# alex-petrenko/megaverse

Measured on NVIDIA H100. Metric: agent obs/sec (whole box), higher is better.
Workload: dtype f32

## Files before the change

### megaverse_b200/capi.py

```python
import ctypes as C
import os

import numpy as np

_PKG = os.path.dirname(os.path.abspath(__file__))
LIB_PATH = os.environ.get("MV_B200_LIB") or os.path.join(_PKG, "libmegaverse_b200.so")
_lib = None

MV_OK, MV_ERR_ARG, MV_ERR_CUDA, MV_ERR_CAPACITY, MV_ERR_STATE = 0, -1, -2, -3, -4
MV_END_NONE, MV_END_TIME, MV_END_SOLVED, MV_END_REQUESTED = 0, 1, 2, 3
MV_SEG_NONE, MV_SEG_STATIC, MV_SEG_TERRAIN, MV_SEG_OBJECT, MV_SEG_AGENT, MV_SEG_REWARD = 0, 1, 2, 3, 4, 5
MAX_OBJECTS, MAX_AGENTS, MAX_CAND = 128, 8, 96
MV_FAULT_ENVELOPE, MV_FAULT_CAND_OVERFLOW = 16, 32
CUDA_STREAM_LEGACY = 0x1


class MegaverseError(RuntimeError):
    def __init__(self, code, msg):
        super().__init__("megaverse_b200 error %d: %s" % (code, msg))
        self.code = code


def lib():
    global _lib
# ... 402 lines not shown
    def stream(self):
        p = C.c_void_p()
        self._ck(lib().mv_stream(self._h, C.byref(p)))
        return p.value

    def get_reward_shaping(self, env, agent):
        keys = (C.c_char_p * 32)()
        vals = (C.c_float * 32)()
        n = C.c_int()
        self._ck(lib().mv_get_reward_shaping(self._h, env, agent, keys, vals, 32, C.byref(n)))
        return {keys[i].decode(): float(vals[i]) for i in range(n.value)}

    def set_reward_shaping(self, env, agent, rs):
        keys = (C.c_char_p * max(1, len(rs)))(*[k.encode() for k in rs])
        vals = (C.c_float * max(1, len(rs)))(*[float(v) for v in rs.values()])
        self._ck(lib().mv_set_reward_shaping(self._h, env, agent, keys, vals, len(rs)))

    def faults(self):
        f = C.c_int32()
        self._ck(lib().mv_faults(self._h, C.byref(f)))
        return f.value

    def fault_word(self):
        f = C.c_int32()
        lib().mv_fault_word.argtypes = [C.c_void_p, C.POINTER(C.c_int32)]
        self._ck(lib().mv_fault_word(self._h, C.byref(f)))
        return f.value

    def kernel_launches(self):
        n = C.c_int64()
        self._ck(lib().mv_kernel_launches(self._h, C.byref(n)))
        return n.value

    def step_profile(self, enable=True, read=True):
        out = np.zeros((self.E, 16), dtype=np.uint32)
        lib().mv_debug_step_profile.argtypes = [C.c_void_p, C.c_void_p, C.c_int]
        self._ck(lib().mv_debug_step_profile(self._h, out.ctypes.data if read else None, 1 if enable else 0))
        return out

    def static_cap(self):
        lib().mv_debug_static_cap.argtypes = [C.c_void_p]
        return int(lib().mv_debug_static_cap(self._h))

    def raster_config(self):
        out = (C.c_int32 * 4)()
        lib().mv_debug_raster_config.argtypes = [C.c_void_p, C.c_void_p]
        self._ck(lib().mv_debug_raster_config(self._h, out))
        return {"grid": out[0], "ctas_per_sm": out[1], "smem": out[2], "bands": out[3]}

    def raster_stats(self, enable=True, read=True):
        out = (C.c_ulonglong * 16)()
        lib().mv_debug_raster_stats.argtypes = [C.c_void_p, C.c_void_p, C.c_int]
        self._ck(lib().mv_debug_raster_stats(self._h, out if read else None, 1 if enable else 0))
        names = ["work_items", "instances", "visible_instances", "items", "clipped_items", "triangles", "batches", "sub_passes", "cyc_head", "cyc_tma_wait", "cyc_instance", "cyc_item", "cyc_tile", "cyc_total"]
        return {n: int(out[i]) for i, n in enumerate(names)}

    def states_create(self, rows):
        sid = C.c_int()
        self._ck(lib().mv_states_create(self._h, int(rows), C.byref(sid)))
        return sid.value

    def states_save(self, store, envs, rows):
        e, r = np.ascontiguousarray(envs, dtype=np.int32), np.ascontiguousarray(rows, dtype=np.int32)
        assert e.size == r.size
        self._ck(lib().mv_states_save(self._h, int(store), e.ctypes.data, r.ctypes.data, e.size))

    def states_load(self, store, rows, envs):
        r, e = np.ascontiguousarray(rows, dtype=np.int32), np.ascontiguousarray(envs, dtype=np.int32)
        assert e.size == r.size
        self._ck(lib().mv_states_load(self._h, int(store), r.ctypes.data, e.ctypes.data, e.size))

    def states_destroy(self, store):
        self._ck(lib().mv_states_destroy(self._h, int(store)))

    def state_row_bytes(self):
        n = C.c_int64()
        self._ck(lib().mv_state_row_bytes(self._h, C.byref(n)))
        return n.value

    def last_kernel_ms(self):
        out = (C.c_float * 2)()
        self._ck(lib().mv_last_kernel_ms(self._h, out))
        return float(out[0]), float(out[1])

    def last_final_ms(self):
        out = C.c_float()
        self._ck(lib().mv_last_final_ms(self._h, C.byref(out)))
        return float(out.value)

    def _dump(self, fn, env, dtype, cap=1 << 16):
        out = np.zeros(cap, dtype=dtype)
        n = getattr(lib(), fn)(self._h, env, out.ctypes.data, cap)
        if n < -8:
            return self._dump(fn, env, dtype, -n)
        if n < 0:
            self._ck(n)
        return out[:n].copy()

    def level(self, env):
        return self._dump("mv_debug_get_level", env, np.int32)

    def state(self, env):
        return self._dump("mv_debug_get_state", env, np.float32)

    def voxels(self, env):
        return self._dump("mv_debug_get_voxels", env, np.int32).reshape(-1, 4)

# ... 107 lines not shown
```

### megaverse_b200/csrc/raster_view.cuh

```cuda
#pragma once
#include "dev_math.cuh"
#include "mesh_tables.inc"
#include "mv_types.h"

namespace mvr {
using namespace dm;

struct __align__(16) TriCover {
    long long C[3];
    int32_t A[3], B[3];
    float z[3];
    float invArea;
    uint32_t key;
    int32_t flags;
    uint32_t bx, by;
};
struct __align__(16) TriShade {
    float rw[3];
    float p[9];
    float n[9];
    float diffuse[3];
};
static_assert(sizeof(TriCover) == 80 && sizeof(TriShade) == 96, "triangle record layout");

#ifndef MV_VIEW_THREADS
#define MV_VIEW_THREADS 256
#endif
#ifndef MV_VIEW_MIN_CTAS
#define MV_VIEW_MIN_CTAS 2
#endif
constexpr int kThreads = MV_VIEW_THREADS;
constexpr int kWarps = kThreads / 32;
#ifndef MV_VIEW_INST_CHUNK
#define MV_VIEW_INST_CHUNK 128
#endif
constexpr int kInstChunk = MV_VIEW_INST_CHUNK;
static_assert(kInstChunk <= kThreads && kInstChunk <= 128, "one thread per instance of a chunk; slow-list entries keep 7 bits of it");
constexpr int kXfWords = 23;
constexpr int kClipVerts = 6;
constexpr int kSmallList = 128;
#ifndef MV_SMALL_AREA
#define MV_SMALL_AREA 4
#endif
constexpr int kSmallArea = MV_SMALL_AREA;
constexpr int kIdxBits = 10;
constexpr uint32_t kStaleIdx = (1u << kIdxBits) - 1u;
constexpr int kMaxTriCap = int(kStaleIdx);
constexpr int kKeyBits = 32 - kIdxBits;
constexpr int kMaxInstancesPerEnv = (1 << (kKeyBits - 7)) - 1;
static_assert(MV_CAPSULE_TRIS <= 128 && MV_SPHERE_TRIS <= 128 && MV_CONE_TRIS <= 128 && MV_CYLINDER_TRIS <= 128, "triangle-in-mesh index needs 7 bits");

constexpr int kVBox = 0, kVCapsule = kVBox + MV_BOX_VERTS, kVSphere = kVCapsule + MV_CAPSULE_VERTS, kVCone = kVSphere + MV_SPHERE_VERTS,
              kVCylinder = kVCone + MV_CONE_VERTS, kMeshVerts = kVCylinder + MV_CYLINDER_VERTS;
constexpr int kICapsule = 0, kISphere = kICapsule + MV_CAPSULE_TRIS * 3, kICone = kISphere + MV_SPHERE_TRIS * 3, kICylinder = kICone + MV_CONE_TRIS * 3,
              kMeshIdx = kICylinder + MV_CYLINDER_TRIS * 3;

struct ViewParams {
    const MvInstance *instances;
    const int32_t *instCounts;
    const float *views;
    int instStride;
    uint8_t *obs;
    float *depth;
    uint16_t *seg;
    uint32_t *workCounter;
    uint32_t counterBase;
    const uint32_t *ready;
    uint32_t readyStamp;
    unsigned long long *stats;
    uint32_t *viewCost;
    uint32_t *order;
    uint32_t *exitCounter;
    unsigned long long *spill;
    int spillStride;
    int viewBase, N;
    int A, W, H;
    int bands, bandRows;
    int triCap;
    float p00, p11, p22, p32;
    const uint8_t *envMask;
    const int32_t *camEnv;
    uint32_t *rangeCount;
    int numEnvs;
};

struct SmemLayout { uint32_t stage, cover, shade, xf, off, frag, small, meshV, meshI, clip, slow, sched, misc, total; };
struct ViewMisc {
    float view[16];
    int32_t counts[8];
    int32_t nTris;
    int32_t nValid;
    int32_t tileCtr;
    uint32_t claim;
    int32_t prefetched;
    int32_t lastCta;
    int32_t wsum[kWarps];
    int32_t nSlow[2];
    uint32_t stat[8];
    alignas(8) unsigned long long bar[2];
    unsigned long long itemStart;
};
__host__ __device__ inline SmemLayout smemLayout(int triCap) {
    SmemLayout L;
    uint32_t o = 0;
    L.stage = o; o += 2u * kInstChunk * uint32_t(sizeof(MvInstance));
    L.cover = o; o += uint32_t(triCap) * uint32_t(sizeof(TriCover));
    L.shade = o; o += uint32_t(triCap) * uint32_t(sizeof(TriShade));
    L.xf = o; o += uint32_t(kXfWords) * kInstChunk * 4u;
    L.off = o; o += (kInstChunk + 4u) * 4u;
    L.frag = o; o += uint32_t(kWarps) * 128u * 8u;
    L.meshV = o; o += uint32_t(kMeshVerts) * 6u * 4u;
    L.meshI = o; o += (uint32_t(kMeshIdx) + 15u) & ~15u;
    L.clip = L.frag;
    L.small = o; o += uint32_t(kWarps) * kSmallList * 2u;
    L.slow = o; o += 2u * kThreads * 2u;
    L.sched = o; o += 256u * 4u;
    L.misc = o; o += (uint32_t(sizeof(ViewMisc)) + 15u) & ~15u;
    L.total = o;
    return L;
}

__device__ __forceinline__ uint32_t smemAddrOf(const void *p) { return uint32_t(__cvta_generic_to_shared(p)); }
__device__ __forceinline__ void mbarInit(unsigned long long *bar, int count) {
    asm volatile("mbarrier.init.shared::cta.b64 [%0], %1;" ::"r"(smemAddrOf(bar)), "r"(count));
    asm volatile("fence.mbarrier_init.release.cluster;" ::: "memory");
}
__device__ __forceinline__ void mbarExpectTx(unsigned long long *bar, uint32_t bytes) {
    asm volatile("mbarrier.arrive.expect_tx.shared::cta.b64 _, [%0], %1;" ::"r"(smemAddrOf(bar)), "r"(bytes) : "memory");
}
__device__ __forceinline__ void bulkG2S(void *dst, const void *src, uint32_t bytes, unsigned long long *bar) {
    asm volatile("cp.async.bulk.shared::cluster.global.mbarrier::complete_tx::bytes [%0], [%1], %2, [%3];" ::"r"(smemAddrOf(dst)), "l"(src), "r"(bytes),
                 "r"(smemAddrOf(bar))
                 : "memory");
}
__device__ __forceinline__ void mbarWait(unsigned long long *bar, uint32_t parity) {
    uint32_t done;
    do {
        asm volatile(
            "{\n"
            ".reg .pred p;\n"
            "mbarrier.try_wait.parity.shared::cta.b64 p, [%1], %2;\n"
            "selp.u32 %0, 1, 0, p;\n"
            "}\n"
            : "=r"(done)
            : "r"(smemAddrOf(bar)), "r"(parity)
            : "memory");
    } while (!done);
}

__constant__ float c_palette[22][3];

struct ClipVert { float cx, cy, cz, cw, px, py, pz, nx, ny, nz; };
static_assert(sizeof(ClipVert) == 40, "ClipVert is ten floats");

__device__ __forceinline__ ClipVert lerpVert(const ClipVert &a, const ClipVert &b, float t) {
    ClipVert o;
    o.cx = a.cx + t * (b.cx - a.cx); o.cy = a.cy + t * (b.cy - a.cy); o.cz = a.cz + t * (b.cz - a.cz); o.cw = a.cw + t * (b.cw - a.cw);
    o.px = a.px + t * (b.px - a.px); o.py = a.py + t * (b.py - a.py); o.pz = a.pz + t * (b.pz - a.pz);
    o.nx = a.nx + t * (b.nx - a.nx); o.ny = a.ny + t * (b.ny - a.ny); o.nz = a.nz + t * (b.nz - a.nz);
    return o;
}
__device__ __forceinline__ int32_t snapSub(float v) { return int32_t(floorf(v * 256.0f + 0.5f)); }

struct SetupCtx {
    TriCover *cover;
    TriShade *shade;
    int32_t *nTris;
    int32_t *nValid;
    int triCap;
    int W, H;
    int rowLo, rowHi;
};
__device__ __forceinline__ int nthFace(unsigned mask, int n) {
    int face = 0, seen = 0;
#pragma unroll
    for (int f = 0; f < 6; ++f) {
        const int bit = int(mask >> f) & 1;
        if (bit && seen == n) face = f;
        seen += bit;
    }
    return face;
}
__device__ __forceinline__ int reserveTris(const SetupCtx &cx, int n) {
    int base;
    asm volatile("atom.shared.add.s32 %0, [%1], %2;" : "=r"(base) : "r"(smemAddrOf(cx.nTris)), "r"(n) : "memory");
    if (base + n <= cx.triCap) return base;
    asm volatile("red.shared.min.s32 [%0], %1;" ::"r"(smemAddrOf(cx.nValid)), "r"(base) : "memory");
    return -1;
}

struct ScreenVert { int32_t sx, sy; float sz, rw; };
__device__ __forceinline__ ScreenVert projectVert(const ClipVert &v, float hw, float hh) {
    ScreenVert o;
    const float r = 1.0f / v.cw;
    o.rw = r;
    o.sx = snapSub((v.cx * r) * hw + hw);
    o.sy = snapSub((v.cy * r) * hh + hh);
    o.sz = v.cz * r;
    return o;
}
__device__ __forceinline__ bool snapOutOfRange(const ScreenVert &a, const ScreenVert &b, const ScreenVert &c) {
    constexpr long long kSnapMax = 1518500249ll;
    const long long x0 = a.sx, x1 = b.sx, x2 = c.sx, y0 = a.sy, y1 = b.sy, y2 = c.sy;
    const long long ax = max(llabs(x0), max(llabs(x1), llabs(x2))), ay = max(llabs(y0), max(llabs(y1), llabs(y2)));
    const long long dx = max(x0, max(x1, x2)) - min(x0, min(x1, x2)), dy = max(y0, max(y1, y2)) - min(y0, min(y1, y2));
    return ax > kSnapMax || ay > kSnapMax || dx >= (1ll << 31) || dy >= (1ll << 31);
}

struct TriBox { long long area2; uint32_t bx, by; };
__device__ __forceinline__ bool triBox(const SetupCtx &cx, const ScreenVert &a, const ScreenVert &b, const ScreenVert &c, TriBox &o) {
    o.area2 = (long long)(b.sx - a.sx) * (long long)(c.sy - a.sy) - (long long)(b.sy - a.sy) * (long long)(c.sx - a.sx);
    if (o.area2 >= 0) return false;
    const int32_t minx = min(a.sx, min(b.sx, c.sx)), maxx = max(a.sx, max(b.sx, c.sx));
    const int32_t miny = min(a.sy, min(b.sy, c.sy)), maxy = max(a.sy, max(b.sy, c.sy));
    const int px0 = max(0, (minx - 128 + 255) >> 8), px1 = min(cx.W - 1, (maxx - 128) >> 8);
    const int py0 = max(0, (miny - 128 + 255) >> 8), py1 = min(cx.H - 1, (maxy - 128) >> 8);
    if (px0 > px1 || py0 > py1) return false;
    if (py0 > cx.rowHi || py1 < cx.rowLo) return false;
    o.bx = uint32_t(px0) | (uint32_t(px1) << 16);
    o.by = uint32_t(py0) | (uint32_t(py1) << 16);
    return true;
}
template <bool FAST>
__device__ __forceinline__ void writeTri(const SetupCtx &cx, int slot, const ClipVert &va, const ClipVert &vb, const ClipVert &vc, const ScreenVert &a,
                                         const ScreenVert &b, const ScreenVert &c, const TriBox &tb, int colorTag, uint32_t key) {
    const int color = colorTag & 0xffff;
    TriCover cv;
    TriShade s;
    const int32_t sxs[3] = {a.sx, b.sx, c.sx}, sys[3] = {a.sy, b.sy, c.sy};
    int tl = 0;
    long long worst = 0;
    const long long wsub = (long long)cx.W * 256, hsub = (long long)cx.H * 256;
#pragma unroll
    for (int e = 0; e < 3; ++e) {
        const int ia = (e + 1) % 3, ib = (e + 2) % 3;
        const long long dx = (long long)sxs[ib] - sxs[ia], dy = (long long)sys[ib] - sys[ia];
        const bool topleft = (dy == 0 && dx < 0) || dy > 0;
        cv.A[e] = int32_t(dy);
        cv.B[e] = int32_t(-dx);
        cv.C[e] = dx * sys[ia] - dy * sxs[ia] - (topleft ? 0 : 1);
        tl |= topleft ? (1 << e) : 0;
        const long long bound = llabs(dy) * wsub + llabs(dx) * hsub + llabs(cv.C[e]);
        worst = bound > worst ? bound : worst;
    }
    cv.z[0] = a.sz; cv.z[1] = b.sz; cv.z[2] = c.sz;
    s.rw[0] = a.rw; s.rw[1] = b.rw; s.rw[2] = c.rw;
    s.p[0] = va.px; s.p[1] = va.py; s.p[2] = va.pz; s.p[3] = vb.px; s.p[4] = vb.py; s.p[5] = vb.pz; s.p[6] = vc.px; s.p[7] = vc.py; s.p[8] = vc.pz;
    s.n[0] = va.nx; s.n[1] = va.ny; s.n[2] = va.nz; s.n[3] = vb.nx; s.n[4] = vb.ny; s.n[5] = vb.nz; s.n[6] = vc.nx; s.n[7] = vc.ny; s.n[8] = vc.nz;
    const bool flat = va.nx == vb.nx && va.ny == vb.ny && va.nz == vb.nz && va.nx == vc.nx && va.ny == vc.ny && va.nz == vc.nz;
    if (FAST && flat) {
        const float inv = rsqrtf(va.nx * va.nx + va.ny * va.ny + va.nz * va.nz);
        s.n[0] = va.nx * inv; s.n[1] = va.ny * inv; s.n[2] = va.nz * inv;
    }
    cv.invArea = 1.0f / float(-tb.area2);
    cv.key = key;
    cv.flags = tl | (worst < (1ll << 30) ? 8 : 0) | (flat ? 16 : 0) | (colorTag & int(0xffff0000u));
    cv.bx = tb.bx;
    cv.by = tb.by;
    s.diffuse[0] = c_palette[color][0]; s.diffuse[1] = c_palette[color][1]; s.diffuse[2] = c_palette[color][2];
    cx.cover[slot] = cv;
    cx.shade[slot] = s;
}

__device__ __forceinline__ void vertPosition(ClipVert &cv, const float mv[12], const float *vp, float p00, float p11, float p22, float p32) {
    { float acc = 0.0f; acc += mv[0] * vp[0]; acc += mv[3] * vp[1]; acc += mv[6] * vp[2]; acc += mv[9] * 1.0f; cv.px = acc; }
    { float acc = 0.0f; acc += mv[1] * vp[0]; acc += mv[4] * vp[1]; acc += mv[7] * vp[2]; acc += mv[10] * 1.0f; cv.py = acc; }
    { float acc = 0.0f; acc += mv[2] * vp[0]; acc += mv[5] * vp[1]; acc += mv[8] * vp[2]; acc += mv[11] * 1.0f; cv.pz = acc; }
    cv.cx = cv.px * p00;
    cv.cy = cv.py * p11;
    cv.cz = cv.pz * p22 + p32;
    cv.cw = -cv.pz;
}
__device__ __forceinline__ void vertNormal(ClipVert &cv, const float nm[9], const float *vp) {
    cv.nx = nm[0] * vp[3] + nm[3] * vp[4] + nm[6] * vp[5];
    cv.ny = nm[1] * vp[3] + nm[4] * vp[4] + nm[7] * vp[5];
    cv.nz = nm[2] * vp[3] + nm[5] * vp[4] + nm[8] * vp[5];
}
__device__ __forceinline__ ClipVert makeVert(const float mv[12], const float nm[9], const float *vp, float p00, float p11, float p22, float p32) {
    ClipVert cv;
    vertPosition(cv, mv, vp, p00, p11, p22, p32);
    vertNormal(cv, nm, vp);
    return cv;
}

__device__ __forceinline__ bool insideNearFar(const ClipVert &v) { return v.cz >= 0.0f && (v.cw - v.cz) >= 0.0f; }
__device__ __forceinline__ unsigned sideOutcode(const ClipVert &v) {
    return (v.cx > v.cw ? 1u : 0u) | (v.cx < -v.cw ? 2u : 0u) | (v.cy > v.cw ? 4u : 0u) | (v.cy < -v.cw ? 8u : 0u);
}

enum SetupResult { kSetupDone = 0, kSetupFull = 1, kSetupClip = 2 };

template <bool FAST, bool RANGE = false>
__device__ __forceinline__ SetupResult setupItem(const SetupCtx &cx, ClipVert &v0, ClipVert &v1, ClipVert &v2, ClipVert &v3, int nTri, const float nm[9], const float *vp0,
                                                 const float *vp1, const float *vp2, const float *vp3, int color, uint32_t keyBase,
                                                 uint32_t *rangeCount = nullptr) {
    if (sideOutcode(v0) & sideOutcode(v1) & sideOutcode(v2) & sideOutcode(v3)) return kSetupDone;
    if (!(insideNearFar(v0) && insideNearFar(v1) && insideNearFar(v2) && insideNearFar(v3))) {
        if (v0.cz < 0.0f && v1.cz < 0.0f && v2.cz < 0.0f && v3.cz < 0.0f) return kSetupDone;
        if ((v0.cw - v0.cz) < 0.0f && (v1.cw - v1.cz) < 0.0f && (v2.cw - v2.cz) < 0.0f && (v3.cw - v3.cz) < 0.0f) return kSetupDone;
        return kSetupClip;
    }
    const float hw = float(cx.W) * 0.5f, hh = float(cx.H) * 0.5f;
    const ScreenVert s0 = projectVert(v0, hw, hh), s1 = projectVert(v1, hw, hh), s2 = projectVert(v2, hw, hh);
    ScreenVert s3 = s2;
    if (nTri == 2) s3 = projectVert(v3, hw, hh);
    TriBox b0, b1;
    const bool vis0 = triBox(cx, s0, s1, s2, b0), vis1 = nTri == 2 && triBox(cx, s0, s2, s3, b1);
    const int n = (vis0 ? 1 : 0) + (vis1 ? 1 : 0);
    auto countWide = [&] {
        const uint32_t wide = (snapOutOfRange(s0, s1, s2) ? 1u : 0u) + (nTri == 2 && snapOutOfRange(s0, s2, s3) ? 1u : 0u);
        if (wide && rangeCount) atomicAdd(rangeCount, wide);
    };
    if (!n) {
        if (RANGE) countWide();
        return kSetupDone;
    }
    int slot = reserveTris(cx, n);
    if (slot < 0) return kSetupFull;
    if (RANGE) countWide();
    vertNormal(v0, nm, vp0); vertNormal(v1, nm, vp1); vertNormal(v2, nm, vp2); vertNormal(v3, nm, vp3);
#pragma unroll 1
    for (int t = 0; t < 2; ++t) {
        if (!(t ? vis1 : vis0)) continue;
        const ClipVert vb = t ? v2 : v1, vc = t ? v3 : v2;
        const ScreenVert sb = t ? s2 : s1, sc = t ? s3 : s2;
        const TriBox tb = t ? b1 : b0;
        writeTri<FAST>(cx, slot++, v0, vb, vc, s0, sb, sc, tb, color, keyBase + uint32_t(t));
    }
    return kSetupDone;
}

__device__ __forceinline__ int clipNearFar(float *bufA, float *bufB, int c, unsigned groupMask) {
    float *src = bufA, *dst = bufB;
    int n = 3;
    for (int plane = 0; plane < 2; ++plane) {
        int m = 0;
        for (int i = 0; i < n; ++i) {
            const int i1 = i + 1 == n ? 0 : i + 1;
            const float az = src[i * 10 + 2], aw = src[i * 10 + 3], bz = src[i1 * 10 + 2], bw = src[i1 * 10 + 3];
            const float da = plane == 0 ? az : aw - az;
            const float db = plane == 0 ? bz : bw - bz;
            const bool ina = da >= 0.0f, inb = db >= 0.0f;
            float a = 0.0f, b = 0.0f;
            if (c < 10) { a = src[i * 10 + c]; b = src[i1 * 10 + c]; }
            if (ina) { if (c < 10) dst[m * 10 + c] = a; ++m; }
            if (ina != inb) {
                float val;
                if (ina) { const float t = da / (da - db); val = a + t * (b - a); }
                else { const float t = db / (db - da); val = b + t * (a - b); }
                if (c < 10) dst[m * 10 + c] = val;
                ++m;
            }
        }
        __syncwarp(groupMask);
        n = m;
        float *sw = src; src = dst; dst = sw;
        if (n < 3) return 0;
    }
    return n;
}

__device__ __forceinline__ bool instanceMayBeVisible(const M4 &mv, float by, float p00, float p11) {
    const float l0 = sqrtf(mv.c[0] * mv.c[0] + mv.c[1] * mv.c[1] + mv.c[2] * mv.c[2]);
    const float l1 = sqrtf(mv.c[4] * mv.c[4] + mv.c[5] * mv.c[5] + mv.c[6] * mv.c[6]);
    const float l2 = sqrtf(mv.c[8] * mv.c[8] + mv.c[9] * mv.c[9] + mv.c[10] * mv.c[10]);
    const float r = (l0 + by * l1 + l2) * 1.001f + 1e-3f;
    const float x = mv.c[12], y = mv.c[13], z = mv.c[14];
    if (-z - 0.01f < -r) return false;
    const float ix = rsqrtf(p00 * p00 + 1.0f), iy = rsqrtf(p11 * p11 + 1.0f);
    const float ax = fabsf(p00), ay = fabsf(p11);
    if ((-ax * x - z) * ix < -r || (ax * x - z) * ix < -r) return false;
    if ((-ay * y - z) * iy < -r || (ay * y - z) * iy < -r) return false;
    return true;
// ... 422 lines not shown

    if (tid == 0) { M.claim = claimWork<ITEMS>(P, total); M.prefetched = 0; }
    for (;;) {
        const long long tc0 = P.stats ? clock64() : 0;
        long long tcWait = 0, tcInst = 0, tcItem = 0;
        __syncthreads();
        const uint32_t claim = M.claim;
        const bool prefetched = M.prefetched != 0;
        if (claim >= total) break;
        const int vrel = int(claim / uint32_t(bands)), band = int(claim - uint32_t(vrel) * uint32_t(bands));
        const int view = P.viewBase + vrel;
        const int env = CAM ? P.camEnv[vrel] : view / P.A;
        const bool live = !CAM || (env >= 0 && env < P.numEnvs);
        const int rowLo = band * P.bandRows, rowHi = min(P.H, rowLo + P.bandRows) - 1;
        const int bandTiles = tilesX * ((rowHi - rowLo + 1) >> 2);
        const MvInstance *inst = P.instances + size_t(env) * size_t(P.instStride);

        if (tid == 0) {
            if (P.ready && !prefetched) {
                const uint32_t *flag = P.ready + env;
                uint32_t v;
                while (true) {
                    asm volatile("ld.acquire.gpu.global.u32 %0, [%1];" : "=r"(v) : "l"(flag) : "memory");
                    if (v == P.readyStamp) break;
                    __nanosleep(200);
                }
                asm volatile("fence.proxy.async;" ::: "memory");
            }
            M.itemStart = (unsigned long long)clock64();
            M.nTris = 0;
            M.nValid = 0x7fffffff;
            M.tileCtr = 0;
            M.nSlow[0] = 0; M.nSlow[1] = 0;
            for (int q = 0; q < 8; ++q) M.stat[q] = 0;
        }
        __syncthreads();
        if (!prefetched) {
            if (tid < 16) M.view[tid] = __ldcg(P.views + size_t(view) * 16 + tid);
            else if (tid < 24) M.counts[tid - 16] = live ? __ldcg(P.instCounts + env * 8 + (tid - 16)) : 0;
            __syncthreads();
        }
        const int nInst = M.counts[1];
        const int nChunks = (nInst + kInstChunk - 1) / kInstChunk;
        if (tid == 0 && nChunks > 0 && !prefetched) {
            const uint32_t bytes = uint32_t(min(nInst, kInstChunk)) * uint32_t(sizeof(MvInstance));
            mbarExpectTx(&M.bar[0], bytes);
            bulkG2S(stage, inst, bytes, &M.bar[0]);
        }
        M4 viewM;
#pragma unroll
        for (int i = 0; i < 16; ++i) viewM.c[i] = M.view[i];

        SetupCtx cx;
        cx.cover = cover; cx.shade = shade; cx.nTris = &M.nTris; cx.nValid = &M.nValid; cx.triCap = P.triCap; cx.W = P.W; cx.H = P.H; cx.rowLo = rowLo; cx.rowHi = rowHi;
        int batch = 0, parity = 0;
        const long long tc1 = P.stats ? clock64() : 0;

        for (int c = 0; c < nChunks; ++c) {
            const int buf = c & 1;
            const int cBase = c * kInstChunk, cCnt = min(kInstChunk, nInst - cBase);
            const long long tw0 = P.stats ? clock64() : 0;
            mbarWait(&M.bar[buf], phase[buf]);
            phase[buf] ^= 1u;
            const long long tw1 = P.stats ? clock64() : 0;
            tcWait += tw1 - tw0;
            if (tid == 0 && c + 1 < nChunks) {
                const int nCnt = min(kInstChunk, nInst - (cBase + kInstChunk));
                const uint32_t bytes = uint32_t(nCnt) * uint32_t(sizeof(MvInstance));
                mbarExpectTx(&M.bar[buf ^ 1], bytes);
                bulkG2S(stage + (buf ^ 1) * kInstChunk, inst + cBase + kInstChunk, bytes, &M.bar[buf ^ 1]);
            }
            int items = 0;
            if (tid < cCnt) {
                const float4 *src = reinterpret_cast<const float4 *>(stage + buf * kInstChunk + tid);
                const float4 c0 = src[0], c1 = src[1], c2 = src[2], c3 = src[3], c4 = src[4];
                M4 model;
                model.c[0] = c0.x; model.c[1] = c0.y; model.c[2] = c0.z; model.c[3] = c0.w;
                model.c[4] = c1.x; model.c[5] = c1.y; model.c[6] = c1.z; model.c[7] = c1.w;
                model.c[8] = c2.x; model.c[9] = c2.y; model.c[10] = c2.z; model.c[11] = c2.w;
                model.c[12] = c3.x; model.c[13] = c3.y; model.c[14] = c3.z; model.c[15] = c3.w;
                const int mesh = __float_as_int(c4.x), color = __float_as_int(c4.y);
                const M4 mv = mul4(viewM, model);
                int meta = mesh;
                if (instanceMayBeVisible(mv, mesh == 1 ? 2.0f : 1.0f, P.p00, P.p11)) {
                    float nm[9];
                    const float det = normalMatrix(mv, nm);
                    const bool mirrored = !(det > 0.0f);
                    if (mirrored) meta |= 1 << 16;
                    if (mesh == 0) {
                        int mask = mirrored ? 63 : 0;
#pragma unroll
                        for (int face = 0; face < 6; ++face) {
                            const float *fn = meshV + (face * 4) * 6 + 3;
                            const float cxv = mv.c[12] + (fn[0] * mv.c[0] + fn[1] * mv.c[4] + fn[2] * mv.c[8]);
                            const float cyv = mv.c[13] + (fn[0] * mv.c[1] + fn[1] * mv.c[5] + fn[2] * mv.c[9]);
                            const float czv = mv.c[14] + (fn[0] * mv.c[2] + fn[1] * mv.c[6] + fn[2] * mv.c[10]);
                            const float nxv = nm[0] * fn[0] + nm[3] * fn[1] + nm[6] * fn[2];
                            const float nyv = nm[1] * fn[0] + nm[4] * fn[1] + nm[7] * fn[2];
                            const float nzv = nm[2] * fn[0] + nm[5] * fn[1] + nm[8] * fn[2];
                            const float d = nxv * cxv + nyv * cyv + nzv * czv;
                            if (!(d > 1e-3f * sqrtf((nxv * nxv + nyv * nyv + nzv * nzv) * (cxv * cxv + cyv * cyv + czv * czv)))) mask |= 1 << face;
                        }
                        items = __popc(mask);
                        meta |= mask << 8;
                    } else {
                        items = mesh == 1 ? MV_CAPSULE_TRIS : (mesh == 2 ? MV_SPHERE_TRIS : (mesh == 3 ? MV_CONE_TRIS : MV_CYLINDER_TRIS));
                    }
                    if (items) {
#pragma unroll
                        for (int col = 0; col < 4; ++col)
#pragma unroll
                            for (int row = 0; row < 3; ++row) xf[(col * 3 + row) * kInstChunk + tid] = mv.c[col * 4 + row];
#pragma unroll
                        for (int q = 0; q < 9; ++q) xf[(12 + q) * kInstChunk + tid] = nm[q];
                        xf[21 * kInstChunk + tid] = __int_as_float(color | (__float_as_int(c4.z) << 16));
                    }
                }
                xf[22 * kInstChunk + tid] = __int_as_float(meta);
                if (P.stats && items) atomicAdd(&M.stat[2], 1u);
            }
            {
                int incl = items;
#pragma unroll
                for (int d = 1; d < 32; d <<= 1) {
                    const int up = __shfl_up_sync(0xffffffffu, incl, d);
                    if (lane >= d) incl += up;
                }
                if (lane == 31) M.wsum[warp] = incl;
                __syncthreads();
                int prefix = 0, totalItems = 0;
#pragma unroll
                for (int w = 0; w < kWarps; ++w) { const int s = M.wsum[w]; if (w < warp) prefix += s; totalItems += s; }
                if (tid < kInstChunk) off[tid] = prefix + incl - items;
                if (tid == 0) off[kInstChunk] = totalItems;
                __syncthreads();
            }
            const int totalItems = off[kInstChunk];
            const long long tw2 = P.stats ? clock64() : 0;
            tcInst += tw2 - tw1;
            if (P.stats && tid == 0) { M.stat[1] += uint32_t(cCnt); M.stat[3] += uint32_t(totalItems); }
            for (int ibase = 0; ibase < totalItems; ibase += kThreads, parity ^= 1) {
                const int j = ibase + tid;
                uint16_t *slowList = slowAll + parity * kThreads;
                if (tid == 0) { M.nSlow[parity ^ 1] = 0; if (P.stats) M.stat[7] += 1; }
                bool pending = j < totalItems, pushed = false, again = false;
                for (;;) {
                    if (pending) {
                        int lo = 0, hi = cCnt - 1;
                        while (lo < hi) {
                            const int mid = (lo + hi + 1) >> 1;
                            if (off[mid] <= j) lo = mid; else hi = mid - 1;
                        }
                        const int i = lo, sub = j - off[i];
                        float mv[12], nm[9];
#pragma unroll
                        for (int q = 0; q < 12; ++q) mv[q] = xf[q * kInstChunk + i];
#pragma unroll
                        for (int q = 0; q < 9; ++q) nm[q] = xf[(12 + q) * kInstChunk + i];
                        const int color = __float_as_int(xf[21 * kInstChunk + i]);
                        const int meta = __float_as_int(xf[22 * kInstChunk + i]);
                        const int mesh = meta & 255;
                        const uint32_t ii = uint32_t(cBase + i);
                        ClipVert cvt[4];
                        const float *vpn[4];
                        int nTri;
                        uint32_t keyBase;
                        bool facesAway = false;
                        if (mesh == 0) {
                            const int face = nthFace(unsigned(meta >> 8) & 63u, sub);
#pragma unroll
                            for (int k = 0; k < 4; ++k) vpn[k] = meshV + (face * 4 + k) * 6;
                            nTri = 2; keyBase = ii * 128u + uint32_t(face) * 2u + 1u;
                        } else {
                            const int vBase = mesh == 1 ? kVCapsule : (mesh == 2 ? kVSphere : (mesh == 3 ? kVCone : kVCylinder));
                            const int iBase = mesh == 1 ? kICapsule : (mesh == 2 ? kISphere : (mesh == 3 ? kICone : kICylinder));
#pragma unroll
                            for (int k = 0; k < 3; ++k) vpn[k] = meshV + (vBase + int(meshI[iBase + sub * 3 + k])) * 6;
                            vpn[3] = vpn[2];
                            nTri = 1; keyBase = ii * 128u + uint32_t(sub) + 1u;
#ifndef MV_NO_MESH_PRECULL
                            if (!(meta & (1 << 16))) {
                                const float t0 = mv[9], t1 = mv[10], t2 = mv[11];
                                const float ex = -(nm[0] * t0 + nm[1] * t1 + nm[2] * t2), ey = -(nm[3] * t0 + nm[4] * t1 + nm[5] * t2), ez = -(nm[6] * t0 + nm[7] * t1 + nm[8] * t2);
                                const float *pa = vpn[0], *pb = vpn[1], *pc = vpn[2];
                                const float ux = pb[0] - pa[0], uy = pb[1] - pa[1], uz = pb[2] - pa[2], vx = pc[0] - pa[0], vy = pc[1] - pa[1], vz = pc[2] - pa[2];
                                const float nx = uy * vz - uz * vy, ny = uz * vx - ux * vz, nz = ux * vy - uy * vx;
                                const float dx = ex - pa[0], dy = ey - pa[1], dz = ez - pa[2];
                                const float sd = nx * dx + ny * dy + nz * dz;
                                facesAway = sd < 0.0f && sd * sd > 4e-4f * ((nx * nx + ny * ny + nz * nz) * (dx * dx + dy * dy + dz * dz));
                            }
#endif
                        }
                        SetupResult res = kSetupDone;
                        if (!facesAway) {
#pragma unroll
                            for (int k = 0; k < 4; ++k) vertPosition(cvt[k], mv, vpn[k], P.p00, P.p11, P.p22, P.p32);
                            res = setupItem<FAST, CAM>(cx, cvt[0], cvt[1], cvt[2], cvt[3], nTri, nm, vpn[0], vpn[1], vpn[2], vpn[3], color, keyBase,
                                                       CAM && band == 0 ? P.rangeCount : nullptr);
                        }
                        pending = res == kSetupFull;
                        if (res == kSetupClip) {
                            int at;
                            asm volatile("atom.shared.add.s32 %0, [%1], 1;" : "=r"(at) : "r"(smemAddrOf(&M.nSlow[parity])) : "memory");
                            slowList[at] = uint16_t(i | (sub << 7));
                            pushed = true;
                        }
                    }
                    const bool any = __syncthreads_or((pending || pushed) ? 1 : 0) || again;
                    pushed = false;
                    if (!any) break;
                    bool slowFull = false;
                    const int nSlow = M.nSlow[parity];
                    if (P.stats && tid == 0 && !again) M.stat[4] += uint32_t(nSlow);
                    for (int sidx = warp; sidx < nSlow; sidx += kWarps) {
                        const int e = slowList[sidx];
                        if (e & 0x8000) continue;
                        const int i = e & 127, sub = (e >> 7) & 127;
                        float mv[12], nm[9];
#pragma unroll
                        for (int q = 0; q < 12; ++q) mv[q] = xf[q * kInstChunk + i];
#pragma unroll
                        for (int q = 0; q < 9; ++q) nm[q] = xf[(12 + q) * kInstChunk + i];
                        const int color = __float_as_int(xf[21 * kInstChunk + i]);
                        const int meta = __float_as_int(xf[22 * kInstChunk + i]);
                        const int mesh = meta & 255;
                        const uint32_t ii = uint32_t(cBase + i);
                        ClipVert *poly0 = clipScratch, *poly1 = clipScratch + kClipVerts, *tmp0 = clipScratch + 2 * kClipVerts, *tmp1 = clipScratch + 3 * kClipVerts;
                        int nSrc;
                        uint32_t keyBase;
                        if (mesh == 0) {
                            const int face = nthFace(unsigned(meta >> 8) & 63u, sub);
                            nSrc = 2; keyBase = ii * 128u + uint32_t(face) * 2u + 1u;
                            if (lane < 4) {
                                const ClipVert v = makeVert(mv, nm, meshV + (face * 4 + lane) * 6, P.p00, P.p11, P.p22, P.p32);
                                if (lane == 0) { poly0[0] = v; poly1[0] = v; }
                                else if (lane == 1) poly0[1] = v;
                                else if (lane == 2) { poly0[2] = v; poly1[1] = v; }
                                else poly1[2] = v;
                            }
                        } else {
                            const int vBase = mesh == 1 ? kVCapsule : (mesh == 2 ? kVSphere : (mesh == 3 ? kVCone : kVCylinder));
                            const int iBase = mesh == 1 ? kICapsule : (mesh == 2 ? kISphere : (mesh == 3 ? kICone : kICylinder));
                            nSrc = 1; keyBase = ii * 128u + uint32_t(sub) + 1u;
                            if (lane < 3) poly0[lane] = makeVert(mv, nm, meshV + (vBase + int(meshI[iBase + sub * 3 + lane])) * 6, P.p00, P.p11, P.p22, P.p32);
                        }
                        __syncwarp();
                        int nv = 0;
                        if ((lane >> 4) < nSrc)
                            nv = clipNearFar(reinterpret_cast<float *>(lane >> 4 ? poly1 : poly0), reinterpret_cast<float *>(lane >> 4 ? tmp1 : tmp0), lane & 15,
                                             0xffffu << (lane & 16));
                        __syncwarp();
                        const int n0 = __shfl_sync(0xffffffffu, nv, 0), n1 = __shfl_sync(0xffffffffu, nv, 16);
                        const int t = lane / 3, k = lane - t * 3 + 1;
                        const ClipVert *pp = t ? poly1 : poly0;
                        bool vis = false, wide = false;
                        TriBox tb;
                        ScreenVert sa, sb, sc;
                        if (lane < 6 && k + 1 < (t ? n1 : n0)) {
                            const float hw = float(P.W) * 0.5f, hh = float(P.H) * 0.5f;
                            sa = projectVert(pp[0], hw, hh); sb = projectVert(pp[k], hw, hh); sc = projectVert(pp[k + 1], hw, hh);
                            vis = triBox(cx, sa, sb, sc, tb);
                            if (CAM) wide = snapOutOfRange(sa, sb, sc);
                        }
                        const unsigned vm = __ballot_sync(0xffffffffu, vis);
                        bool done = true;
                        if (vm) {
                            int base = 0;
                            if (lane == 0) base = reserveTris(cx, __popc(vm));
                            base = __shfl_sync(0xffffffffu, base, 0);
                            if (base < 0) done = false;
                            else if (vis) writeTri<FAST>(cx, base + __popc(vm & ((1u << lane) - 1u)), pp[0], pp[k], pp[k + 1], sa, sb, sc, tb, color, keyBase + uint32_t(t));
                        }
                        if (done) { if (lane == 0) slowList[sidx] = uint16_t(e | 0x8000); }
                        else slowFull = true;
                        if (CAM && done && band == 0 && P.rangeCount) {
                            const unsigned wm = __ballot_sync(0xffffffffu, wide);
                            if (lane == 0 && wm) atomicAdd(P.rangeCount, uint32_t(__popc(wm)));
                        }
                        __syncwarp();
                    }
                    if (!__syncthreads_or((pending || slowFull) ? 1 : 0)) break;
                    tilePass<FAST, SEG>(P, min(M.nTris, M.nValid), spill, view, rowLo, bandTiles, batch, false);
                    if (P.stats && tid == 0) M.stat[5] += uint32_t(min(M.nTris, M.nValid));
                    ++batch;
                    again = true;
                    __syncthreads();
                    if (tid == 0) { M.nTris = 0; M.nValid = 0x7fffffff; M.tileCtr = 0; }
                    __syncthreads();
                }
            }
            __syncthreads();
            if (P.stats) tcItem += clock64() - tw2;
        }
        const long long tc2 = P.stats ? clock64() : 0;
        if (tid == 0) {
            const uint32_t nc = claimWork<ITEMS>(P, total);
            int pre = 0;
            if (nc < total) {
                const int nview = P.viewBase + int(nc / uint32_t(bands)), nenv = CAM ? P.camEnv[nview] : nview / P.A;
                const bool nlive = !CAM || (nenv >= 0 && nenv < P.numEnvs);
                bool ready = true;
                if (P.ready) {
                    uint32_t v;
                    asm volatile("ld.acquire.gpu.global.u32 %0, [%1];" : "=r"(v) : "l"(P.ready + nenv) : "memory");
                    ready = v == P.readyStamp;
                    if (ready) asm volatile("fence.proxy.async;" ::: "memory");
                }
                if (ready) {
                    float vm[16];
                    int32_t cn[8];
#pragma unroll
                    for (int q = 0; q < 16; ++q) vm[q] = __ldcg(P.views + size_t(nview) * 16 + q);
#pragma unroll
                    for (int q = 0; q < 8; ++q) cn[q] = nlive ? __ldcg(P.instCounts + nenv * 8 + q) : 0;
#pragma unroll
                    for (int q = 0; q < 16; ++q) M.view[q] = vm[q];
#pragma unroll
                    for (int q = 0; q < 8; ++q) M.counts[q] = cn[q];
                    if (cn[1] > 0) {
                        const uint32_t bytes = uint32_t(min(cn[1], kInstChunk)) * uint32_t(sizeof(MvInstance));
                        mbarExpectTx(&M.bar[0], bytes);
                        bulkG2S(stage, P.instances + size_t(nenv) * size_t(P.instStride), bytes, &M.bar[0]);
                    }
                    pre = 1;
                }
            }
            M.claim = nc; M.prefetched = pre;
        }
        if (live) {
            tilePass<FAST, SEG>(P, min(M.nTris, M.nValid), spill, view, rowLo, bandTiles, batch, true);
        } else {
            const size_t px0 = (size_t(view) * P.H + size_t(rowLo)) * P.W;
            for (int q = tid; q < ((rowHi - rowLo + 1) * P.W) >> 2; q += kThreads) {
                const size_t p = px0 + size_t(q) * 4;
                *reinterpret_cast<uint4 *>(P.obs + p * 4) = make_uint4(0u, 0u, 0u, 0u);
                if (P.depth) *reinterpret_cast<float4 *>(P.depth + p) = make_float4(0.0f, 0.0f, 0.0f, 0.0f);
                if (SEG) *reinterpret_cast<uint2 *>(P.seg + p) = make_uint2(0u, 0u);
            }
        }
        __syncthreads();
        if (P.viewCost && tid == 0) P.viewCost[claim] = uint32_t(min((unsigned long long)clock64() - M.itemStart, 0xffffffffull * 16ull) >> 4);
        if (P.stats && tid < 8) {
            unsigned long long v = M.stat[tid];
            if (tid == 0) v = 1;
            if (tid == 5) v += (unsigned long long)min(M.nTris, M.nValid);
            if (tid == 6) v = (unsigned long long)(batch + 1);
            atomicAdd(P.stats + tid, v);
            if (tid == 0) {
                const long long tc3 = clock64();
                atomicAdd(P.stats + 8, (unsigned long long)(tc1 - tc0)); atomicAdd(P.stats + 9, (unsigned long long)tcWait);
                atomicAdd(P.stats + 10, (unsigned long long)tcInst); atomicAdd(P.stats + 11, (unsigned long long)tcItem);
                atomicAdd(P.stats + 12, (unsigned long long)(tc3 - tc2)); atomicAdd(P.stats + 13, (unsigned long long)(tc3 - tc0));
            }
        }
    }
    if (P.viewCost) {
        if (tid == 0) {
            __threadfence();
            M.lastCta = atomicAdd(P.exitCounter, 1u) == gridDim.x - 1u ? 1 : 0;
        }
        __syncthreads();
        if (M.lastCta) {
            __threadfence();
            uint32_t *bins = reinterpret_cast<uint32_t *>(smem + L.sched);
            const int E = P.N / P.A;
            uint32_t *costS = reinterpret_cast<uint32_t *>(smem + L.cover);
            const int capS = int((L.xf - L.cover) / 4u);
            const bool inSmem = E <= capS;
            if (inSmem) {
                for (int e = tid; e < E; e += kThreads) costS[e] = 0u;
                __syncthreads();
                const uint32_t perEnv = uint32_t(P.A) * uint32_t(P.bands);
                const int items = int(total);
                for (int v0 = tid; v0 < items; v0 += 4 * kThreads) {
                    uint32_t c[4];
#pragma unroll
                    for (int q = 0; q < 4; ++q) { const int v = v0 + q * kThreads; c[q] = v < items ? __ldcg(P.viewCost + v) : 0u; }
#pragma unroll
                    for (int q = 0; q < 4; ++q) { const int v = v0 + q * kThreads; if (v < items) atomicAdd(&costS[uint32_t(v) / perEnv], c[q]); }
                }
                __syncthreads();
            }
            auto envCost = [&](int e) {
                if (inSmem) return costS[e];
                uint32_t c = 0u;
                const int perEnv = P.A * P.bands;
                for (int a = 0; a < perEnv; ++a) c += __ldcg(P.viewCost + e * perEnv + a);
                return c;
            };
            uint32_t mx = 1u;
            for (int e = tid; e < E; e += kThreads) mx = max(mx, envCost(e));
#pragma unroll
            for (int d = 16; d; d >>= 1) mx = max(mx, __shfl_xor_sync(0xffffffffu, mx, d));
            if (lane == 0) M.wsum[warp] = int32_t(mx);
            for (int b = tid; b < 256; b += kThreads) bins[b] = 0u;
            __syncthreads();
#pragma unroll
            for (int w = 0; w < kWarps; ++w) mx = max(mx, uint32_t(M.wsum[w]));
            const float scale = 255.0f / float(mx);
            auto keyOf = [&](int e) { return 255 - min(255, int(float(envCost(e)) * scale)); };
            for (int e = tid; e < E; e += kThreads) atomicAdd(&bins[keyOf(e)], 1u);
            __syncthreads();
            {
                const int per = (256 + kThreads - 1) / kThreads, b0 = min(256, tid * per), b1 = min(256, b0 + per);
                uint32_t sum = 0u;
// ... 24 lines not shown
```

Baseline: 2.916 million.

## Precompute per-batch capsule/sphere vertex transforms into a shared-memory table

```diff
diff --git a/megaverse_b200/capi.py b/megaverse_b200/capi.py
--- a/megaverse_b200/capi.py
+++ b/megaverse_b200/capi.py
@@ -478,7 +478,8 @@
         out = (C.c_ulonglong * 16)()
         lib().mv_debug_raster_stats.argtypes = [C.c_void_p, C.c_void_p, C.c_int]
         self._ck(lib().mv_debug_raster_stats(self._h, out if read else None, 1 if enable else 0))
-        names = ["work_items", "instances", "visible_instances", "items", "clipped_items", "triangles", "batches", "sub_passes", "cyc_head", "cyc_tma_wait", "cyc_instance", "cyc_item", "cyc_tile", "cyc_total"]
+        names = ["work_items", "instances", "visible_instances", "items", "clipped_items", "triangles", "batches", "sub_passes", "cyc_head", "cyc_tma_wait", "cyc_instance", "cyc_item", "cyc_tile", "cyc_total",
+                 "mesh_tris_table", "mesh_tris_own"]
         return {n: int(out[i]) for i, n in enumerate(names)}
 
     def states_create(self, rows):
diff --git a/megaverse_b200/csrc/raster_view.cuh b/megaverse_b200/csrc/raster_view.cuh
--- a/megaverse_b200/csrc/raster_view.cuh
+++ b/megaverse_b200/csrc/raster_view.cuh
@@ -54,6 +54,11 @@
               kVCylinder = kVCone + MV_CONE_VERTS, kMeshVerts = kVCylinder + MV_CYLINDER_VERTS;
 constexpr int kICapsule = 0, kISphere = kICapsule + MV_CAPSULE_TRIS * 3, kICone = kISphere + MV_SPHERE_TRIS * 3, kICylinder = kICone + MV_CONE_TRIS * 3,
               kMeshIdx = kICylinder + MV_CYLINDER_TRIS * 3;
+__device__ __forceinline__ int meshVertBase(int mesh) { return mesh == 1 ? kVCapsule : (mesh == 2 ? kVSphere : (mesh == 3 ? kVCone : kVCylinder)); }
+__device__ __forceinline__ int tableVerts(int mesh) { return mesh == 1 ? MV_CAPSULE_VERTS : (mesh == 2 ? MV_SPHERE_VERTS : 0); }
+constexpr int kTableMinFree = 8;
+constexpr int kVertOffShift = 17;
+static_assert(kInstChunk * MV_CAPSULE_VERTS < (1 << (31 - kVertOffShift)) && MV_CAPSULE_VERTS >= MV_SPHERE_VERTS, "vertex offsets fit the meta word");
 
 struct ViewParams {
     const MvInstance *instances;
@@ -97,6 +102,8 @@
     int32_t wsum[kWarps];
     int32_t nSlow[2];
     uint32_t stat[8];
+    int16_t listCap;
+    int16_t vertLo;
     alignas(8) unsigned long long bar[2];
     unsigned long long itemStart;
 };
@@ -167,7 +174,7 @@
     TriShade *shade;
     int32_t *nTris;
     int32_t *nValid;
-    int triCap;
+    uint32_t listCap;
     int W, H;
     int rowLo, rowHi;
 };
@@ -184,7 +191,9 @@
 __device__ __forceinline__ int reserveTris(const SetupCtx &cx, int n) {
     int base;
     asm volatile("atom.shared.add.s32 %0, [%1], %2;" : "=r"(base) : "r"(smemAddrOf(cx.nTris)), "r"(n) : "memory");
-    if (base + n <= cx.triCap) return base;
+    int cap;
+    asm volatile("ld.shared.s16 %0, [%1];" : "=r"(cap) : "r"(cx.listCap) : "memory");
+    if (base + n <= cap) return base;
     asm volatile("red.shared.min.s32 [%0], %1;" ::"r"(smemAddrOf(cx.nValid)), "r"(base) : "memory");
     return -1;
 }
@@ -290,20 +299,38 @@
 
 enum SetupResult { kSetupDone = 0, kSetupFull = 1, kSetupClip = 2 };
 
+struct __align__(16) VertRec { int32_t sx, sy; float sz, rw; float px, py, pz; uint32_t flags; };
+static_assert(sizeof(VertRec) == 32, "vertex record layout");
+constexpr uint32_t kInNear = 16u, kInFar = 32u, kBehindNear = 64u, kBeyondFar = 128u;
+__device__ __forceinline__ VertRec makeRec(const ClipVert &v, float hw, float hh) {
+    const ScreenVert s = projectVert(v, hw, hh);
+    VertRec r;
+    r.sx = s.sx; r.sy = s.sy; r.sz = s.sz; r.rw = s.rw;
+    r.px = v.px; r.py = v.py; r.pz = v.pz;
+    r.flags = sideOutcode(v) | (v.cz >= 0.0f ? kInNear : 0u) | ((v.cw - v.cz) >= 0.0f ? kInFar : 0u) | (v.cz < 0.0f ? kBehindNear : 0u) |
+              ((v.cw - v.cz) < 0.0f ? kBeyondFar : 0u);
+    return r;
+}
+__device__ __forceinline__ ScreenVert screenOf(const VertRec &r) { return ScreenVert{r.sx, r.sy, r.sz, r.rw}; }
+__device__ __forceinline__ ClipVert shadeVert(const VertRec &r, const float nm[9], const float *vp) {
+    ClipVert v;
+    v.cx = v.cy = v.cz = v.cw = 0.0f;
+    v.px = r.px; v.py = r.py; v.pz = r.pz;
+    vertNormal(v, nm, vp);
+    return v;
+}
+
 template <bool FAST, bool RANGE = false>
-__device__ __forceinline__ SetupResult setupItem(const SetupCtx &cx, ClipVert &v0, ClipVert &v1, ClipVert &v2, ClipVert &v3, int nTri, const float nm[9], const float *vp0,
-                                                 const float *vp1, const float *vp2, const float *vp3, int color, uint32_t keyBase,
-                                                 uint32_t *rangeCount = nullptr) {
-    if (sideOutcode(v0) & sideOutcode(v1) & sideOutcode(v2) & sideOutcode(v3)) return kSetupDone;
-    if (!(insideNearFar(v0) && insideNearFar(v1) && insideNearFar(v2) && insideNearFar(v3))) {
-        if (v0.cz < 0.0f && v1.cz < 0.0f && v2.cz < 0.0f && v3.cz < 0.0f) return kSetupDone;
-        if ((v0.cw - v0.cz) < 0.0f && (v1.cw - v1.cz) < 0.0f && (v2.cw - v2.cz) < 0.0f && (v3.cw - v3.cz) < 0.0f) return kSetupDone;
+__device__ __forceinline__ SetupResult setupItem(const SetupCtx &cx, const VertRec &r0, const VertRec &r1, const VertRec &r2, const VertRec &r3, int nTri,
+                                                 const float *nmCol, const float *meshV, int vo0, int vo1, int vo2, int vo3, int color,
+                                                 uint32_t keyBase, uint32_t *rangeCount = nullptr) {
+    const uint32_t all = r0.flags & r1.flags & r2.flags & r3.flags;
+    if (all & 15u) return kSetupDone;
+    if ((all & (kInNear | kInFar)) != (kInNear | kInFar)) {
+        if (all & (kBehindNear | kBeyondFar)) return kSetupDone;
         return kSetupClip;
     }
-    const float hw = float(cx.W) * 0.5f, hh = float(cx.H) * 0.5f;
-    const ScreenVert s0 = projectVert(v0, hw, hh), s1 = projectVert(v1, hw, hh), s2 = projectVert(v2, hw, hh);
-    ScreenVert s3 = s2;
-    if (nTri == 2) s3 = projectVert(v3, hw, hh);
+    const ScreenVert s0 = screenOf(r0), s1 = screenOf(r1), s2 = screenOf(r2), s3 = screenOf(r3);
     TriBox b0, b1;
     const bool vis0 = triBox(cx, s0, s1, s2, b0), vis1 = nTri == 2 && triBox(cx, s0, s2, s3, b1);
     const int n = (vis0 ? 1 : 0) + (vis1 ? 1 : 0);
@@ -318,7 +345,11 @@
     int slot = reserveTris(cx, n);
     if (slot < 0) return kSetupFull;
     if (RANGE) countWide();
-    vertNormal(v0, nm, vp0); vertNormal(v1, nm, vp1); vertNormal(v2, nm, vp2); vertNormal(v3, nm, vp3);
+    float nm[9];
+#pragma unroll
+    for (int q = 0; q < 9; ++q) nm[q] = nmCol[q * kInstChunk];
+    const ClipVert v0 = shadeVert(r0, nm, meshV + vo0 * 6), v1 = shadeVert(r1, nm, meshV + vo1 * 6), v2 = shadeVert(r2, nm, meshV + vo2 * 6),
+                   v3 = shadeVert(r3, nm, meshV + vo3 * 6);
 #pragma unroll 1
     for (int t = 0; t < 2; ++t) {
         if (!(t ? vis1 : vis0)) continue;
@@ -847,8 +878,16 @@
         for (int i = 0; i < 16; ++i) viewM.c[i] = M.view[i];
 
         SetupCtx cx;
-        cx.cover = cover; cx.shade = shade; cx.nTris = &M.nTris; cx.nValid = &M.nValid; cx.triCap = P.triCap; cx.W = P.W; cx.H = P.H; cx.rowLo = rowLo; cx.rowHi = rowHi;
+        cx.cover = cover; cx.shade = shade; cx.nTris = &M.nTris; cx.nValid = &M.nValid; cx.listCap = smemAddrOf(&M.listCap); cx.W = P.W; cx.H = P.H; cx.rowLo = rowLo; cx.rowHi = rowHi;
         int batch = 0, parity = 0;
+        auto drawBatch = [&] {
+            tilePass<FAST, SEG>(P, min(M.nTris, M.nValid), spill, view, rowLo, bandTiles, batch, false);
+            if (P.stats && tid == 0) M.stat[5] += uint32_t(min(M.nTris, M.nValid));
+            ++batch;
+            __syncthreads();
+            if (tid == 0) { M.nTris = 0; M.nValid = 0x7fffffff; M.tileCtr = 0; }
+            __syncthreads();
+        };
         const long long tc1 = P.stats ? clock64() : 0;
 
         for (int c = 0; c < nChunks; ++c) {
@@ -865,7 +904,7 @@
                 mbarExpectTx(&M.bar[buf ^ 1], bytes);
                 bulkG2S(stage + (buf ^ 1) * kInstChunk, inst + cBase + kInstChunk, bytes, &M.bar[buf ^ 1]);
             }
-            int items = 0;
+            int items = 0, verts = 0, meta = 0;
             if (tid < cCnt) {
                 const float4 *src = reinterpret_cast<const float4 *>(stage + buf * kInstChunk + tid);
                 const float4 c0 = src[0], c1 = src[1], c2 = src[2], c3 = src[3], c4 = src[4];
@@ -876,7 +915,7 @@
                 model.c[12] = c3.x; model.c[13] = c3.y; model.c[14] = c3.z; model.c[15] = c3.w;
                 const int mesh = __float_as_int(c4.x), color = __float_as_int(c4.y);
                 const M4 mv = mul4(viewM, model);
-                int meta = mesh;
+                meta = mesh;
                 if (instanceMayBeVisible(mv, mesh == 1 ? 2.0f : 1.0f, P.p00, P.p11)) {
                     float nm[9];
                     const float det = normalMatrix(mv, nm);
@@ -900,6 +939,7 @@
                         meta |= mask << 8;
                     } else {
                         items = mesh == 1 ? MV_CAPSULE_TRIS : (mesh == 2 ? MV_SPHERE_TRIS : (mesh == 3 ? MV_CONE_TRIS : MV_CYLINDER_TRIS));
+                        verts = tableVerts(mesh);
                     }
                     if (items) {
 #pragma unroll
@@ -911,11 +951,11 @@
                         xf[21 * kInstChunk + tid] = __int_as_float(color | (__float_as_int(c4.z) << 16));
                     }
                 }
-                xf[22 * kInstChunk + tid] = __int_as_float(meta);
                 if (P.stats && items) atomicAdd(&M.stat[2], 1u);
             }
             {
-                int incl = items;
+                const int own = items | (verts << 16);
+                int incl = own;
 #pragma unroll
                 for (int d = 1; d < 32; d <<= 1) {
                     const int up = __shfl_up_sync(0xffffffffu, incl, d);
@@ -926,11 +966,22 @@
                 int prefix = 0, totalItems = 0;
 #pragma unroll
                 for (int w = 0; w < kWarps; ++w) { const int s = M.wsum[w]; if (w < warp) prefix += s; totalItems += s; }
-                if (tid < kInstChunk) off[tid] = prefix + incl - items;
-                if (tid == 0) off[kInstChunk] = totalItems;
+                const int excl = prefix + incl - own;
+                if (tid < kInstChunk) off[tid] = excl & 0xffff;
+                if (tid < cCnt) xf[22 * kInstChunk + tid] = __int_as_float(meta | ((excl >> 16) << kVertOffShift));
+                if (tid == 0) off[kInstChunk] = totalItems & 0xffff;
                 __syncthreads();
             }
             const int totalItems = off[kInstChunk];
+            auto metaOf = [&](int i) { return __float_as_int(xf[22 * kInstChunk + i]); };
+            auto instanceOf = [&](int item) {
+                int lo = 0, hi = cCnt - 1;
+                while (lo < hi) {
+                    const int mid = (lo + hi + 1) >> 1;
+                    if (off[mid] <= item) lo = mid; else hi = mid - 1;
+                }
+                return lo;
+            };
             const long long tw2 = P.stats ? clock64() : 0;
             tcInst += tw2 - tw1;
             if (P.stats && tid == 0) { M.stat[1] += uint32_t(cCnt); M.stat[3] += uint32_t(totalItems); }
@@ -938,46 +989,67 @@
                 const int j = ibase + tid;
                 uint16_t *slowList = slowAll + parity * kThreads;
                 if (tid == 0) { M.nSlow[parity ^ 1] = 0; if (P.stats) M.stat[7] += 1; }
+                {
+                    const int iLo = instanceOf(ibase), iHi = instanceOf(min(ibase + kThreads, totalItems) - 1);
+                    const int vLo = metaOf(iLo) >> kVertOffShift, metaHi = metaOf(iHi);
+                    const int nVerts = (metaHi >> kVertOffShift) - vLo + tableVerts(metaHi & 255);
+                    const int need = (nVerts + 2) / 3;
+                    int cap = P.triCap;
+                    if (nVerts > 0 && M.nTris + need <= P.triCap - kTableMinFree) {
+                        cap = P.triCap - need;
+                        VertRec *table = reinterpret_cast<VertRec *>(shade + cap);
+                        const float hw = float(P.W) * 0.5f, hh = float(P.H) * 0.5f;
+                        for (int v = tid; v < nVerts; v += kThreads) {
+                            const int g = vLo + v;
+                            int lo = iLo, hi = iHi;
+                            while (lo < hi) {
+                                const int mid = (lo + hi + 1) >> 1;
+                                if ((metaOf(mid) >> kVertOffShift) <= g) lo = mid; else hi = mid - 1;
+                            }
+                            const int meta = metaOf(lo);
+                            float mv[12];
+#pragma unroll
+                            for (int q = 0; q < 12; ++q) mv[q] = xf[q * kInstChunk + lo];
+                            ClipVert c;
+                            vertPosition(c, mv, meshV + (meshVertBase(meta & 255) + g - (meta >> kVertOffShift)) * 6, P.p00, P.p11, P.p22, P.p32);
+                            table[v] = makeRec(c, hw, hh);
+                        }
+                    }
+                    if (tid == 0) { M.listCap = int16_t(cap); M.vertLo = int16_t(vLo); }
+                    __syncthreads();
+                }
                 bool pending = j < totalItems, pushed = false, again = false;
                 for (;;) {
                     if (pending) {
-                        int lo = 0, hi = cCnt - 1;
-                        while (lo < hi) {
-                            const int mid = (lo + hi + 1) >> 1;
-                            if (off[mid] <= j) lo = mid; else hi = mid - 1;
-                        }
-                        const int i = lo, sub = j - off[i];
-                        float mv[12], nm[9];
-#pragma unroll
-                        for (int q = 0; q < 12; ++q) mv[q] = xf[q * kInstChunk + i];
-#pragma unroll
-                        for (int q = 0; q < 9; ++q) nm[q] = xf[(12 + q) * kInstChunk + i];
+                        const int i = instanceOf(j), sub = j - off[i];
                         const int color = __float_as_int(xf[21 * kInstChunk + i]);
-                        const int meta = __float_as_int(xf[22 * kInstChunk + i]);
+                        const int meta = metaOf(i);
                         const int mesh = meta & 255;
                         const uint32_t ii = uint32_t(cBase + i);
-                        ClipVert cvt[4];
-                        const float *vpn[4];
-                        int nTri;
+                        int vo[4];
+                        int vBase = 0, nTri;
                         uint32_t keyBase;
                         bool facesAway = false;
                         if (mesh == 0) {
                             const int face = nthFace(unsigned(meta >> 8) & 63u, sub);
 #pragma unroll
-                            for (int k = 0; k < 4; ++k) vpn[k] = meshV + (face * 4 + k) * 6;
+                            for (int k = 0; k < 4; ++k) vo[k] = face * 4 + k;
                             nTri = 2; keyBase = ii * 128u + uint32_t(face) * 2u + 1u;
                         } else {
-                            const int vBase = mesh == 1 ? kVCapsule : (mesh == 2 ? kVSphere : (mesh == 3 ? kVCone : kVCylinder));
+                            vBase = meshVertBase(mesh);
                             const int iBase = mesh == 1 ? kICapsule : (mesh == 2 ? kISphere : (mesh == 3 ? kICone : kICylinder));
 #pragma unroll
-                            for (int k = 0; k < 3; ++k) vpn[k] = meshV + (vBase + int(meshI[iBase + sub * 3 + k])) * 6;
-                            vpn[3] = vpn[2];
+                            for (int k = 0; k < 3; ++k) vo[k] = vBase + int(meshI[iBase + sub * 3 + k]);
+                            vo[3] = vo[2];
                             nTri = 1; keyBase = ii * 128u + uint32_t(sub) + 1u;
 #ifndef MV_NO_MESH_PRECULL
                             if (!(meta & (1 << 16))) {
-                                const float t0 = mv[9], t1 = mv[10], t2 = mv[11];
+                                float nm[9];
+#pragma unroll
+                                for (int q = 0; q < 9; ++q) nm[q] = xf[(12 + q) * kInstChunk + i];
+                                const float t0 = xf[9 * kInstChunk + i], t1 = xf[10 * kInstChunk + i], t2 = xf[11 * kInstChunk + i];
                                 const float ex = -(nm[0] * t0 + nm[1] * t1 + nm[2] * t2), ey = -(nm[3] * t0 + nm[4] * t1 + nm[5] * t2), ez = -(nm[6] * t0 + nm[7] * t1 + nm[8] * t2);
-                                const float *pa = vpn[0], *pb = vpn[1], *pc = vpn[2];
+                                const float *pa = meshV + vo[0] * 6, *pb = meshV + vo[1] * 6, *pc = meshV + vo[2] * 6;
                                 const float ux = pb[0] - pa[0], uy = pb[1] - pa[1], uz = pb[2] - pa[2], vx = pc[0] - pa[0], vy = pc[1] - pa[1], vz = pc[2] - pa[2];
                                 const float nx = uy * vz - uz * vy, ny = uz * vx - ux * vz, nz = ux * vy - uy * vx;
                                 const float dx = ex - pa[0], dy = ey - pa[1], dz = ez - pa[2];
@@ -988,10 +1060,30 @@
                         }
                         SetupResult res = kSetupDone;
                         if (!facesAway) {
-#pragma unroll
-                            for (int k = 0; k < 4; ++k) vertPosition(cvt[k], mv, vpn[k], P.p00, P.p11, P.p22, P.p32);
-                            res = setupItem<FAST, CAM>(cx, cvt[0], cvt[1], cvt[2], cvt[3], nTri, nm, vpn[0], vpn[1], vpn[2], vpn[3], color, keyBase,
-                                                       CAM && band == 0 ? P.rangeCount : nullptr);
+                            VertRec rv[4];
+                            const int cap = M.listCap;
+                            const bool fromTable = tableVerts(mesh) && cap < P.triCap;
+                            if (fromTable) {
+                                const VertRec *tv = reinterpret_cast<const VertRec *>(shade + cap) + ((meta >> kVertOffShift) - M.vertLo - vBase);
+#pragma unroll
+                                for (int k = 0; k < 3; ++k) rv[k] = tv[vo[k]];
+                                rv[3] = rv[2];
+                            } else {
+                                float mv[12];
+#pragma unroll
+                                for (int q = 0; q < 12; ++q) mv[q] = xf[q * kInstChunk + i];
+                                const float hw = float(P.W) * 0.5f, hh = float(P.H) * 0.5f;
+#pragma unroll
+                                for (int k = 0; k < 4; ++k) {
+                                    if (k == 3 && mesh != 0) { rv[3] = rv[2]; break; }
+                                    ClipVert c;
+                                    vertPosition(c, mv, meshV + vo[k] * 6, P.p00, P.p11, P.p22, P.p32);
+                                    rv[k] = makeRec(c, hw, hh);
+                                }
+                            }
+                            if (P.stats && mesh != 0 && !again) atomicAdd(&M.stat[fromTable ? 0 : 6], 1u);
+                            res = setupItem<FAST, CAM>(cx, rv[0], rv[1], rv[2], rv[3], nTri, xf + 12 * kInstChunk + i, meshV, vo[0], vo[1], vo[2], vo[3], color,
+                                                       keyBase, CAM && band == 0 ? P.rangeCount : nullptr);
                         }
                         pending = res == kSetupFull;
                         if (res == kSetupClip) {
@@ -1075,13 +1167,8 @@
                         __syncwarp();
                     }
                     if (!__syncthreads_or((pending || slowFull) ? 1 : 0)) break;
-                    tilePass<FAST, SEG>(P, min(M.nTris, M.nValid), spill, view, rowLo, bandTiles, batch, false);
-                    if (P.stats && tid == 0) M.stat[5] += uint32_t(min(M.nTris, M.nValid));
-                    ++batch;
+                    drawBatch();
                     again = true;
-                    __syncthreads();
-                    if (tid == 0) { M.nTris = 0; M.nValid = 0x7fffffff; M.tileCtr = 0; }
-                    __syncthreads();
                 }
             }
             __syncthreads();
@@ -1146,6 +1233,7 @@
                 atomicAdd(P.stats + 8, (unsigned long long)(tc1 - tc0)); atomicAdd(P.stats + 9, (unsigned long long)tcWait);
                 atomicAdd(P.stats + 10, (unsigned long long)tcInst); atomicAdd(P.stats + 11, (unsigned long long)tcItem);
                 atomicAdd(P.stats + 12, (unsigned long long)(tc3 - tc2)); atomicAdd(P.stats + 13, (unsigned long long)(tc3 - tc0));
+                atomicAdd(P.stats + 14, (unsigned long long)M.stat[0]); atomicAdd(P.stats + 15, (unsigned long long)M.stat[6]);
             }
         }
     }
```

Result: slower. 2.795 million (median of 6 runs) (-4.2%).
